# XiYe20/VPTR

Measured on AMD Instinct MI355X. Metric: predicted frames/sec (train step) NAR KTH 10->10 @64x64, higher is better.
Workload: dtype bf16x3 (split-bf16 MFMA, fp32 accumulate/storage); 1 GPU; K64: KTH 64x64x1 10->10, VPTREnc/Dec(528, Tanh, reflect) + VPTRFormerNAR(4 enc + 8 dec, d=528, 8 heads, ws 4, dropout 0.10), single_iter of train_NAR.py, random-init weights; per_gpu_batch=16, global_batch=16, frames_per_clip=10, parallelism=dp1, launch=hipGraph, dec_weight_grads=True, frozen_encoder_convs=winograd F(4x4,3x3), 36 strided-batch P16 products per convolution

## Files before the change

### vptr_amd/csrc/gemm_p16.hip

```cpp
#include "gemm_shared.h"

#include <atomic>

typedef __attribute__((ext_vector_type(4))) short s16x4;
typedef __attribute__((ext_vector_type(8))) short s16x8;

constexpr int P16_STAGE = 40 * 1024;

#define P16_GLDS(laddr, gptr) \
  asm volatile("s_mov_b32 m0, %0\n\tglobal_load_lds_dwordx4 %1, off" ::"s"(__builtin_amdgcn_readfirstlane(laddr)), "v"(gptr) : "memory")

__global__ __launch_bounds__(256) void to_p16_kernel(const float* __restrict__ x, unsigned char* __restrict__ out, int64_t n4) {
  for (int64_t i = (int64_t)blockIdx.x * 256 + threadIdx.x; i < n4; i += (int64_t)gridDim.x * 256) {
    const float4 v = reinterpret_cast<const float4*>(x)[i];
    vptr_p16_store4(out, i * 4, v);
  }
}
extern "C" int vptr_to_p16(const float* x, void* out, int64_t rows, int C, vptr_stream_t stream) {
  VPTR_CHECK(x && out && rows > 0 && C > 0 && C % 16 == 0, "to_p16: C must be a positive multiple of 16 (got %d)", C);
  VPTR_CHECK(((reinterpret_cast<uintptr_t>(x) | reinterpret_cast<uintptr_t>(out)) & 15) == 0, "to_p16: pointers must be 16-byte aligned");
  const int64_t n4 = rows * C / 4;
  to_p16_kernel<<<(unsigned)hmin64((n4 + 255) / 256, 16384), 256, 0, (hipStream_t)stream>>>(x, reinterpret_cast<unsigned char*>(out), n4);
  VPTR_LAUNCH_CHECK();
  return 0;
// ... 132 lines not shown

  f32x4 acc[2][6];
#pragma unroll
  for (int mi = 0; mi < 2; ++mi)
#pragma unroll
    for (int ni = 0; ni < 6; ++ni) acc[mi][ni] = (f32x4){0.f, 0.f, 0.f, 0.f};
  int offAh[2], offBh[6];
  const int ch = (lq >> 1) * 4 + (lq & 1);
#pragma unroll
  for (int mi = 0; mi < 2; ++mi) {
    const int r = wm * 32 + mi * 16 + lr, f = (r >> 1) & 7;
    offAh[mi] = r * 128 + ((ch ^ f) << 4);
  }
#pragma unroll
  for (int ni = 0; ni < 6; ++ni) {
    const int r = (wn * 6 + ni) * 16 + lr, f = (r >> 1) & 7;
    offBh[ni] = 16384 + r * 128 + ((ch ^ f) << 4);
  }
  const int nkt = nk * nseg;
  if (NST == 2) issue(0, 0);
  for (int kt = 0; kt < nkt; ++kt) {
    if (NST == 2) __builtin_amdgcn_s_waitcnt(0x0f70);
    __syncthreads();
    if (NST == 2 && kt + 1 < nkt) issue(kt + 1, (kt + 1) & 1);
    const unsigned char* st = p16_smem + (kt & (NST - 1)) * P16_STAGE;
    bf16x8 ah[2], al[2];
#pragma unroll
    for (int mi = 0; mi < 2; ++mi) {
      ah[mi] = *reinterpret_cast<const bf16x8*>(st + offAh[mi]);
      al[mi] = *reinterpret_cast<const bf16x8*>(st + (offAh[mi] ^ 32));
    }
    if (ktail) {
      const int sg = (int)(kt >= nk) + (int)(kt >= 2 * nk);
      if (kt - sg * nk == nk - 1 && lq >= 2) {
#pragma unroll
        for (int mi = 0; mi < 2; ++mi) {
          ah[mi] = (bf16x8){0, 0, 0, 0, 0, 0, 0, 0};
          al[mi] = (bf16x8){0, 0, 0, 0, 0, 0, 0, 0};
        }
      }
    }
    bf16x8 bh[2], bl[2];
    bh[0] = *reinterpret_cast<const bf16x8*>(st + offBh[0]);
    bl[0] = *reinterpret_cast<const bf16x8*>(st + (offBh[0] ^ 32));
#pragma unroll
    for (int ni = 0; ni < 6; ++ni) {
      if (ni == 5 && wn == 1) break;
      if (ni + 1 < 6 && !(ni + 1 == 5 && wn == 1)) {
        bh[(ni + 1) & 1] = *reinterpret_cast<const bf16x8*>(st + offBh[ni + 1]);
        bl[(ni + 1) & 1] = *reinterpret_cast<const bf16x8*>(st + (offBh[ni + 1] ^ 32));
      }
      __builtin_amdgcn_sched_barrier(0);
#pragma unroll
      for (int mi = 0; mi < 2; ++mi) {
        acc[mi][ni] = __builtin_amdgcn_mfma_f32_16x16x32_bf16(al[mi], bh[ni & 1], acc[mi][ni], 0, 0, 0);
        acc[mi][ni] = __builtin_amdgcn_mfma_f32_16x16x32_bf16(ah[mi], bl[ni & 1], acc[mi][ni], 0, 0, 0);
        acc[mi][ni] = __builtin_amdgcn_mfma_f32_16x16x32_bf16(ah[mi], bh[ni & 1], acc[mi][ni], 0, 0, 0);
      }
      __builtin_amdgcn_sched_barrier(0);
    }
  }
  constexpr bool LEAN = EPI != 0;
  if (LEAN) {
    __syncthreads();
    gemm_epilogue_rows_halves_batched<NFN, EPI>(p, mb, acc, reinterpret_cast<float*>(p16_smem), m0, n0, wm, wn, lr, lq, tid, true, false);
  } else if (NST == 4 && !p.atomic && epi_vec_ok(p)) {
    __syncthreads();
    gemm_epilogue_rows_halves_batched<NFN, 0>(p, mb, acc, reinterpret_cast<float*>(p16_smem), m0, n0, wm, wn, lr, lq, tid, true, false);
  } else if (!p.atomic && epi_vec_ok(p)) {
    __syncthreads();
    gemm_epilogue_rows_halves<NFN>(p, mb, acc, reinterpret_cast<float*>(p16_smem), m0, n0, wm, wn, lr, lq, tid, true, false);
  } else {
    gemm_epilogue_serial<NFN>(p, mb, acc, m0, n0, wm, wn, lr, lq, true, p.atomic != 0);
  }
}

__device__ __forceinline__ bf16x8 p16_tr_frag(const unsigned char* st, const int off, const int rb0) {
  const s16x4 a = __builtin_amdgcn_ds_read_tr16_b64_v4i16((__attribute__((address_space(3))) s16x4*)(st + off + rb0));
  const s16x4 b = __builtin_amdgcn_ds_read_tr16_b64_v4i16((__attribute__((address_space(3))) s16x4*)(st + off + (128 - rb0)));
  const s16x8 c = __builtin_shufflevector(a, b, 0, 1, 2, 3, 4, 5, 6, 7);
  return __builtin_bit_cast(bf16x8, c);
}

struct WgSync {
  int* cnt;
  int base;
  int n;
  bool live;
};

template <int SYNC, int MI>
__device__ __forceinline__ void wgrad_p16_tile(const vptr_gemm_desc& p, const int tile, unsigned char* p16_smem, WgSync& sy) {
  constexpr int NW = 8, BN = 176, WM = NW / 2, TR = 16 * MI * WM;
  constexpr int PA = TR / 8 / NW, PB = 24 / NW;
  constexpr int AREG = TR * 128, STG = AREG + 24 * 1024;
  const int NG = p.M, KX = p.N, T = p.K;
  const int tiles_n = (KX + BN - 1) / BN;
  const int m0 = (tile / tiles_n) * TR, n0 = (tile % tiles_n) * BN;
  const int tid = threadIdx.x, lane = tid & 63, wave = tid >> 6;
  const int wm = wave % WM, wn = wave / WM, lr = lane & 15, lq = lane >> 4;
  const int nk = (T + 31) >> 5;
  const int64_t pg = p.lda * 4, px = p.ldb * 4;
  const unsigned char* Gb = reinterpret_cast<const unsigned char*>(p.A);
  const unsigned char* Xb = reinterpret_cast<const unsigned char*>(p.B);

  int colA[PA], colB[PB], trow[PA + PB];
  {
    const int ms = lane >> 4, half = lane & 1, t = (lane & 15) >> 1;
#pragma unroll
    for (int i = 0; i < PA; ++i) {
      const int u = wave + NW * i;
      const int gran = min((m0 >> 4) + (u >> 2) * 2 + (ms >> 1), (NG >> 4) - 1);
      colA[i] = gran * 64 + (ms & 1) * 32 + half * 16;
      trow[i] = (u & 3) * 8 + t;
    }
#pragma unroll
    for (int i = 0; i < PB; ++i) {
      const int v = wave + NW * i;
      const int gran = min((n0 >> 4) + (v >> 2) * 2 + (ms >> 1), (KX >> 4) - 1);
      colB[i] = gran * 64 + (ms & 1) * 32 + half * 16;
      trow[PA + i] = (v & 3) * 8 + t;
    }
  }
  auto issue = [&](const int kt, const int stage) {
    const int t0 = kt * 32;
#pragma unroll
    for (int i = 0; i < PA; ++i)
      P16_GLDS((uint32_t)(stage * STG + (wave + NW * i) * 1024), Gb + (int64_t)min(t0 + trow[i], T - 1) * pg + colA[i]);
#pragma unroll
    for (int i = 0; i < PB; ++i)
      P16_GLDS((uint32_t)(stage * STG + AREG + (wave + NW * i) * 1024), Xb + (int64_t)min(t0 + trow[PA + i], T - 1) * px + colB[i]);
  };

  f32x4 acc[MI][6];
#pragma unroll
  for (int mi = 0; mi < MI; ++mi)
#pragma unroll
    for (int ni = 0; ni < 6; ++ni) acc[mi][ni] = (f32x4){0.f, 0.f, 0.f, 0.f};
  const int lane_off = lq * 1024 + (lr >> 2) * 32 + (lr & 3) * 8;
  const int rb0 = (lq & 1) * 128;
  int offA[MI], offB[6];
#pragma unroll
  for (int mi = 0; mi < MI; ++mi) {
    const int f = wm * MI + mi;
    offA[mi] = (f >> 1) * 4096 + (f & 1) * 512 + lane_off;
  }
#pragma unroll
  for (int ni = 0; ni < 6; ++ni) {
    const int f = wn * 6 + ni;
    offB[ni] = AREG + (f >> 1) * 4096 + (f & 1) * 512 + lane_off;
  }
  const bool flip = p.d_transposed != 0;
  const bool want_rowsum = !flip && p.a_rowsum != nullptr && n0 == 0 && wn == 1;
  const int f0 = (NG - m0 + 15) >> 4;
  const bool colsum_wave = flip && p.a_rowsum != nullptr && f0 < TR / 16 && wm == f0 / MI;
  const int cmi = f0 - wm * MI;
  const __bf16 one = (__bf16)1.0f, zero = (__bf16)0.0f;
  const bf16x8 ones = {one, one, one, one, one, one, one, one};
  const bf16x8 zeros = {zero, zero, zero, zero, zero, zero, zero, zero};
  const bool ttail = (T & 31) != 0;
  const bool rows_live = m0 + wm * (16 * MI) < NG;

  issue(0, 0);
  for (int kt = 0; kt < nk; ++kt) {
    if (SYNC > 0 && kt > 0 && (kt & (SYNC / 2 - 1)) == 0 && threadIdx.x == 0) {
      const int ph = kt & (SYNC - 1);
      if (ph == 0) __hip_atomic_fetch_add(sy.cnt, 1, __ATOMIC_RELAXED, __HIP_MEMORY_SCOPE_AGENT);
      else if (kt > SYNC && sy.live) {
        const int target = sy.base + (kt / SYNC) * sy.n;
        int spins = 0;
        while (__hip_atomic_load(sy.cnt, __ATOMIC_RELAXED, __HIP_MEMORY_SCOPE_AGENT) < target) {
          if (++spins > 3000) {
            sy.live = false;
            __hip_atomic_fetch_add(sy.cnt + 48, 1, __ATOMIC_RELAXED, __HIP_MEMORY_SCOPE_AGENT);
            break;
          }
          __builtin_amdgcn_s_sleep(8);
        }
      }
    }
    __builtin_amdgcn_s_waitcnt(0x0f70);
    __syncthreads();
    if (kt + 1 < nk) issue(kt + 1, (kt + 1) & 1);
    if (!rows_live && !colsum_wave) continue;
    const unsigned char* st = p16_smem + (kt & 1) * STG;
    bf16x8 ah[MI], al[MI];
#pragma unroll
    for (int mi = 0; mi < MI; ++mi) {
      ah[mi] = p16_tr_frag(st, offA[mi], rb0);
      al[mi] = p16_tr_frag(st, offA[mi] + 256, rb0);
    }
    if (colsum_wave) {
#pragma unroll
      for (int mi = 0; mi < MI; ++mi)
        if (mi == cmi) { ah[mi] = ones; al[mi] = zeros; }
    }
    if (ttail && kt == nk - 1) {
      const int tv = T - kt * 32;
#pragma unroll
      for (int e = 0; e < 8; ++e) {
        const int tok = 8 * lq + 4 * ((e >> 2) ^ (lq & 1)) + (e & 3);
        if (tok >= tv) {
#pragma unroll
          for (int mi = 0; mi < MI; ++mi) { ah[mi][e] = zero; al[mi][e] = zero; }
        }
      }
    }
    bf16x8 bh[2], bl[2];
    bh[0] = p16_tr_frag(st, offB[0], rb0);
    bl[0] = p16_tr_frag(st, offB[0] + 256, rb0);
#pragma unroll
    for (int ni = 0; ni < 6; ++ni) {
      if (ni == 5 && wn == 1 && !want_rowsum) break;
      if (ni + 1 < 6) {
        if (ni + 1 == 5 && wn == 1) {
          bh[(ni + 1) & 1] = ones;
          bl[(ni + 1) & 1] = zeros;
        } else {
          bh[(ni + 1) & 1] = p16_tr_frag(st, offB[ni + 1], rb0);
          bl[(ni + 1) & 1] = p16_tr_frag(st, offB[ni + 1] + 256, rb0);
        }
      }
      __builtin_amdgcn_sched_barrier(0);
#pragma unroll
      for (int mi = 0; mi < MI; ++mi) {
        acc[mi][ni] = __builtin_amdgcn_mfma_f32_16x16x32_bf16(al[mi], bh[ni & 1], acc[mi][ni], 0, 0, 0);
        acc[mi][ni] = __builtin_amdgcn_mfma_f32_16x16x32_bf16(ah[mi], bl[ni & 1], acc[mi][ni], 0, 0, 0);
        acc[mi][ni] = __builtin_amdgcn_mfma_f32_16x16x32_bf16(ah[mi], bh[ni & 1], acc[mi][ni], 0, 0, 0);
      }
      __builtin_amdgcn_sched_barrier(0);
    }
  }
  const float alpha = p.alpha;
#pragma unroll
  for (int ni = 0; ni < 6; ++ni) {
    const int nf = wn * 6 + ni, col = n0 + nf * 16 + lr;
    if (nf < 11 && col < KX) {
#pragma unroll
      for (int mi = 0; mi < MI; ++mi)
#pragma unroll
        for (int r = 0; r < 4; ++r) {
          const int row = m0 + (wm * MI + mi) * 16 + lq * 4 + r;
          if (row < NG) {
            float* dst = flip ? p.D + (int64_t)col * p.ldd + row : p.D + (int64_t)row * p.ldd + col;
            if (p.atomic) unsafeAtomicAdd(dst, acc[mi][ni][r] * alpha);
            else *dst = acc[mi][ni][r] * alpha;
          }
        }
    }
  }
  if (colsum_wave && lq == 0) {
#pragma unroll
    for (int ni = 0; ni < 6; ++ni) {
      const int nf = wn * 6 + ni, col = n0 + nf * 16 + lr;
      if (nf < 11 && col < KX) {
        float cs = 0.f;
#pragma unroll
        for (int mi = 0; mi < MI; ++mi)
          if (mi == cmi) cs = acc[mi][ni][0];
        unsafeAtomicAdd(p.a_rowsum + col, cs * alpha);
      }
    }
  }
  if (want_rowsum && lr == 0) {
#pragma unroll
    for (int mi = 0; mi < MI; ++mi)
#pragma unroll
      for (int r = 0; r < 4; ++r) {
        const int row = m0 + (wm * MI + mi) * 16 + lq * 4 + r;
        if (row < NG) unsafeAtomicAdd(p.a_rowsum + row, acc[mi][5][r] * alpha);
      }
  }
}


template <int NSTAGE, int TAG = 0, int NW = 8, int MI = 16 / NW>
__global__ __launch_bounds__(64 * NW, MI == 2 ? 4 : 2) void vptr_wgrad_p16_kernel(const vptr_gemm_desc* __restrict__ descs, const int* __restrict__ tile_start,
                                                                            const int count) {
  static_assert(NSTAGE == 2 && NW == 8, "two stages, eight waves");
  extern __shared__ __attribute__((aligned(1024))) unsigned char p16_smem[];
  const int lg = xcd_logical_block();
  int lo = 0, hi = count - 1;
  while (lo < hi) {
    const int mid = (lo + hi + 1) >> 1;
    if (tile_start[mid] <= lg) lo = mid;
    else hi = mid - 1;
  }
  WgSync none = {nullptr, 0, 0, false};
  wgrad_p16_tile<0, MI>(descs[lo], lg - tile_start[lo], p16_smem, none);
}

__device__ int g_wgrad_sync_ws[8 * 64];
template <int S, int NW = 8, int MI = 16 / NW, int NST = 2>
__global__ __launch_bounds__(64 * NW, MI == 2 ? 4 : 2) void vptr_wgrad_p16_sync_kernel(const vptr_gemm_desc* __restrict__ descs, const int* __restrict__ tile_start,
                                                                const int count, const int total_tiles) {
  static_assert(NST == 2 && NW == 8, "two stages, eight waves");
  extern __shared__ __attribute__((aligned(1024))) unsigned char p16_smem[];
  int* const ws = g_wgrad_sync_ws;
  const int xcd = blockIdx.x & 7, slot = blockIdx.x >> 3, slots = gridDim.x >> 3;
  const int xq = total_tiles >> 3, xr = total_tiles & 7;
  const int first = xcd * xq + min(xcd, xr), mine = xq + (xcd < xr ? 1 : 0);
  const int nk = (descs[0].K + 31) >> 5;
  const int per_tile = (nk - 1) / S;
  WgSync sy = {ws + xcd * 64, 0, 0, true};
  for (int r = 0; r * slots + slot < mine; ++r) {
    const int lg = first + r * slots + slot;
    int lo = 0, hi = count - 1;
    while (lo < hi) {
      const int mid = (lo + hi + 1) >> 1;
      if (tile_start[mid] <= lg) lo = mid;
      else hi = mid - 1;
    }
    sy.base = r * slots * per_tile;
    sy.n = min(slots, mine - r * slots);
    if (r > 0) __syncthreads();
    wgrad_p16_tile<S, MI>(descs[lo], lg - tile_start[lo], p16_smem, sy);
  }
  if (threadIdx.x == 0) {
    int* done = ws + xcd * 64 + 32;
    if (__hip_atomic_fetch_add(done, 1, __ATOMIC_RELAXED, __HIP_MEMORY_SCOPE_AGENT) == slots - 1) {
      __hip_atomic_store(ws + xcd * 64, 0, __ATOMIC_RELAXED, __HIP_MEMORY_SCOPE_AGENT);
      __hip_atomic_store(done, 0, __ATOMIC_RELAXED, __HIP_MEMORY_SCOPE_AGENT);
    }
  }
}

__global__ void wgrad_sync_stats_kernel(int* __restrict__ out) {
  if (threadIdx.x < 8) out[threadIdx.x] = g_wgrad_sync_ws[threadIdx.x * 64 + 48];
}
extern "C" int vptr_wgrad_sync_stats(int* out_dev, vptr_stream_t stream) {
  VPTR_CHECK(out_dev != nullptr, "wgrad_sync_stats: null output");
// ... 31 lines not shown
  if (d.alpha == 0.f) d.alpha = 1.f;
  if (d.batch < 1) d.batch = 1;
  if (d.ksegs < 1) d.ksegs = 1;
  const bool strided = d.batch_stride_d != 0;
  if (strided)
    VPTR_CHECK(d.ksegs == 1 && d.batch <= 4096 && !d.Dpre && !d.residual && !d.atomic && !d.batch_accum && !d.frame_stats && !d.act_grad_src && !d.rowscale &&
                   !d.colscale && d.dropout_p == 0.f && d.act == VPTR_ACT_NONE && !d.act_after &&
                   ((d.batch_stride_a | d.batch_stride_b | d.batch_stride_d) & 15) == 0 && d.batch_stride_a >= 0 && d.batch_stride_b >= 0 && d.batch_stride_d > 0,
               "vptr_gemm(p16): a strided batch takes bias / alpha only and strides that are non-negative multiples of 16");
  VPTR_CHECK((strided || d.batch <= 3) && d.ksegs <= 3 && (d.batch == 1 || d.ksegs == 1), "vptr_gemm(p16): at most 3 batch members or 3 K segments");
  uintptr_t bits = reinterpret_cast<uintptr_t>(d.A) | reinterpret_cast<uintptr_t>(d.B);
  const int extra = strided ? 0 : (d.batch > 1 ? d.batch : d.ksegs) - 1;
  if (extra >= 1) {
    VPTR_CHECK(d.A_x1 && d.B_x1, "vptr_gemm(p16): member / segment 1 needs A_x1, B_x1");
    bits |= reinterpret_cast<uintptr_t>(d.A_x1) | reinterpret_cast<uintptr_t>(d.B_x1);
  }
  if (extra >= 2) {
    VPTR_CHECK(d.A_x2 && d.B_x2, "vptr_gemm(p16): member / segment 2 needs A_x2, B_x2");
    bits |= reinterpret_cast<uintptr_t>(d.A_x2) | reinterpret_cast<uintptr_t>(d.B_x2);
  }
  VPTR_CHECK((bits & 63) == 0, "vptr_gemm(p16): operands must be 64-byte aligned (whole granules)");
  if (d.batch > 1 && !strided) {
    VPTR_CHECK(d.D_x1 && (d.batch < 3 || d.D_x2) && !d.Dpre && !d.residual && !d.atomic, "vptr_gemm(p16): bad batch members");
    if (d.alpha_x1 == 0.f) d.alpha_x1 = 1.f;
    if (d.alpha_x2 == 0.f) d.alpha_x2 = 1.f;
  }
  if (d.rowscale) VPTR_CHECK(d.rs_div >= 1 && d.rs_mod >= 1, "vptr_gemm: rowscale needs rs_div, rs_mod >= 1");
  if (d.dropout_p > 0.f) VPTR_CHECK(d.seed_dev != nullptr && d.dropout_p < 1.f, "vptr_gemm: dropout needs seed_dev and p < 1");
  if (d.d_p16)
    VPTR_CHECK(!d.atomic && d.N % 16 == 0 && d.ldd % 16 == 0 && (d.ldr & 3) == 0 &&
                   ((reinterpret_cast<uintptr_t>(d.D) | reinterpret_cast<uintptr_t>(d.D_x1) | reinterpret_cast<uintptr_t>(d.D_x2)) & 63) == 0 &&
                   ((reinterpret_cast<uintptr_t>(d.residual) | reinterpret_cast<uintptr_t>(d.bias) | reinterpret_cast<uintptr_t>(d.colscale) |
                     reinterpret_cast<uintptr_t>(d.Dpre) | reinterpret_cast<uintptr_t>(d.bias_x1) | reinterpret_cast<uintptr_t>(d.bias_x2)) & 15) == 0,
               "vptr_gemm(p16): a P16 output needs N, ldd multiples of 16, 64-byte aligned D and 16-byte aligned epilogue operands, no atomics");
  static bool attr_set = false;
  if (!attr_set) {
    if (!p16_reserve_lds<0>() || !p16_reserve_lds<1>() || !p16_reserve_lds<2>() || !p16_reserve_lds<3>() || !p16_reserve_lds<4>()) {
      vptr_set_error("vptr_gemm(p16): cannot reserve %d bytes of LDS", 4 * P16_STAGE);
      return -1;
    }
    attr_set = true;
  }
  const int tiles = ((d.M + GBM - 1) / GBM) * ((d.N + 175) / 176) * d.batch;
  uintptr_t ebits = reinterpret_cast<uintptr_t>(d.D) | reinterpret_cast<uintptr_t>(d.residual) | reinterpret_cast<uintptr_t>(d.bias);
  if (d.batch > 1 && !strided) ebits |= reinterpret_cast<uintptr_t>(d.D_x1) | reinterpret_cast<uintptr_t>(d.D_x2) | reinterpret_cast<uintptr_t>(d.bias_x1) | reinterpret_cast<uintptr_t>(d.bias_x2);
  const bool lean = !d.colscale && !d.Dpre && !d.rowscale && d.act == VPTR_ACT_NONE && d.dropout_p == 0.f && !d.act_after && !d.atomic &&
                    (ebits & 15) == 0 && (d.N & 3) == 0 && (d.ldd & 3) == 0 && (d.ldr & 3) == 0;
  const bool lean3 = !lean && !d.colscale && !d.Dpre && (d.rowscale || d.dropout_p > 0.f) && d.act == VPTR_ACT_NONE &&
                     !d.act_after && !d.atomic && !d.frame_stats && (ebits & 15) == 0 && (d.N & 3) == 0 && (d.ldd & 3) == 0 && (d.ldr & 3) == 0;
  const bool lean4 = !lean && !lean3 && !d.colscale && !d.rowscale && !d.residual && !d.act_after && !d.atomic &&
                     d.act != VPTR_ACT_NONE && !d.act_grad_src && !d.frame_stats && d.batch == 1 && !d.batch_accum &&
                     ((ebits | reinterpret_cast<uintptr_t>(d.Dpre)) & 15) == 0 && (d.N & 3) == 0 && (d.ldd & 3) == 0;
  const bool lone = tiles <= vptr_cu_count();
  if (d.frame_stats)
    VPTR_CHECK(d.frame_rows >= 64 && d.frame_rows % 64 == 0 && d.M % 64 == 0 && !d.act_grad_src && lean && d.batch == 1,
               "vptr_gemm(p16): frame_stats needs frame_rows %% 64 == 0, M %% 64 == 0 and a plain launch (bias / alpha / residual only)");
  if (d.act_grad_src) {
    VPTR_CHECK(!d.colscale && !d.Dpre && !d.rowscale && !d.residual && !d.bias && !d.act_after && !d.atomic && d.batch == 1 && d.ksegs == 1 &&
                   d.act != VPTR_ACT_NONE && ((ebits | reinterpret_cast<uintptr_t>(d.act_grad_src)) & 15) == 0 && (d.N & 3) == 0 && (d.ldd & 3) == 0,
               "vptr_gemm(p16): act_grad_src combines with alpha / dropout / P16 output only and needs 16-byte aligned operands, N, ldd multiples of 4");
    p16_launch<2>(d, tiles, lone, st);
    return 0;
  }
  if (d.batch_accum)
    VPTR_CHECK(lean && d.batch > 1 && !d.d_p16 && (d.batch_accum >> d.batch) == 0, "vptr_gemm(p16): batch_accum is an option of plain fp32-output batch launches");
  if (lean4) p16_launch<4>(d, tiles, lone, st);
  else if (lean3) p16_launch<3>(d, tiles, lone, st);
  else if (lean) p16_launch<1>(d, tiles, lone, st);
  else p16_launch<0>(d, tiles, lone, st);
  return 0;
}

static std::atomic<int> g_wgrad_launches[5];
extern "C" int vptr_wgrad_kernel_counts(int* out_host, int n) {
  VPTR_CHECK(out_host != nullptr && n >= 1 && n <= 5, "wgrad_kernel_counts: n must be 1 .. 5 (got %d)", n);
  for (int i = 0; i < n; ++i) out_host[i] = g_wgrad_launches[i].load(std::memory_order_relaxed);
  return 0;
}

int vptr_wgrad_p16_launch(const vptr_gemm_desc* proto, const vptr_gemm_desc* descs_dev, const int* tile_start_dev, int count, int total_tiles,
                          hipStream_t st) {
  VPTR_CHECK(proto->b_mode == VPTR_B_P16T && proto->precision == 3, "vptr_gemm_grouped(p16): both operands token-major P16, precision 3");
  VPTR_CHECK(proto->split_k >= -3, "vptr_gemm_grouped(p16): unknown split_k code %d (include/vptr_hip.h)", proto->split_k);
  constexpr int STG256 = 256 * 128 + 24 * 1024;
  static int sync = -1;
  if (sync < 0) {
    if (hipFuncSetAttribute(reinterpret_cast<const void*>(&vptr_wgrad_p16_kernel<2>), hipFuncAttributeMaxDynamicSharedMemorySize, 2 * P16_STAGE) != hipSuccess ||
        hipFuncSetAttribute(reinterpret_cast<const void*>(&vptr_wgrad_p16_kernel<2, 1>), hipFuncAttributeMaxDynamicSharedMemorySize, 2 * P16_STAGE) != hipSuccess ||
        hipFuncSetAttribute(reinterpret_cast<const void*>(&vptr_wgrad_p16_kernel<2, 0, 8, 4>), hipFuncAttributeMaxDynamicSharedMemorySize, 2 * STG256) != hipSuccess) {
      vptr_set_error("vptr_gemm_grouped(p16): cannot reserve LDS");
      return -1;
    }
    const char* e = getenv("VPTR_WGRAD_SYNC");
    sync = !(e && atoi(e) == 0);
    int per_cu = 0;
    if (sync && (hipFuncSetAttribute(reinterpret_cast<const void*>(&vptr_wgrad_p16_sync_kernel<16>), hipFuncAttributeMaxDynamicSharedMemorySize, 2 * P16_STAGE) != hipSuccess ||
                 hipFuncSetAttribute(reinterpret_cast<const void*>(&vptr_wgrad_p16_sync_kernel<16, 8, 4>), hipFuncAttributeMaxDynamicSharedMemorySize, 2 * STG256) != hipSuccess ||
                 hipOccupancyMaxActiveBlocksPerMultiprocessor(&per_cu, vptr_wgrad_p16_sync_kernel<16>, GNT, 2 * P16_STAGE) != hipSuccess || per_cu < 2))
      sync = 0;
  }
  const int cus = vptr_cu_count();
  if (proto->split_k == -2 || proto->split_k == -3) {
    VPTR_CHECK(proto->atomic, "vptr_gemm_grouped(p16): 256-row tiles accumulate with atomics only");
    if (proto->split_k == -2 && sync && total_tiles >= 512 && cus > 0 && cus % 8 == 0) {
      vptr_wgrad_p16_sync_kernel<16, 8, 4><<<cus, GNT, 2 * STG256, st>>>(descs_dev, tile_start_dev, count, total_tiles);
      g_wgrad_launches[4].fetch_add(1, std::memory_order_relaxed);
    } else {
      vptr_wgrad_p16_kernel<2, 0, 8, 4><<<total_tiles, GNT, 2 * STG256, st>>>(descs_dev, tile_start_dev, count);
      g_wgrad_launches[3].fetch_add(1, std::memory_order_relaxed);
    }
    return 0;
  }
  if (sync && proto->split_k == -1 && proto->atomic && total_tiles >= 1024 && cus > 0 && cus % 4 == 0) {
    vptr_wgrad_p16_sync_kernel<16><<<2 * cus, GNT, 2 * P16_STAGE, st>>>(descs_dev, tile_start_dev, count, total_tiles);
    g_wgrad_launches[2].fetch_add(1, std::memory_order_relaxed);
  } else if (!proto->atomic) {
    vptr_wgrad_p16_kernel<2, 1><<<total_tiles, GNT, 2 * P16_STAGE, st>>>(descs_dev, tile_start_dev, count);
    g_wgrad_launches[1].fetch_add(1, std::memory_order_relaxed);
  } else {
    vptr_wgrad_p16_kernel<2><<<total_tiles, GNT, 2 * P16_STAGE, st>>>(descs_dev, tile_start_dev, count);
    g_wgrad_launches[0].fetch_add(1, std::memory_order_relaxed);
  }
  return 0;
}
```

### vptr_amd/ops/__init__.py

```python
from .core import (
    ACT_NONE, ACT_GELU, ACT_RELU, ACT_LRELU, PAD_MODES, _Config, config, set_deterministic, _direct_apply, _seed_state, _seed_scope,
    _dev_key, _master_seed, new_seed_scope, seed_tensor, manual_seed, DROPPATH_SITE0, droppath_scales, _c, gemm_raw, _Profiling,
    profiling, gemm_nfn, A_P16, B_P16, A_P16T, B_P16T, p16_ok, to_p16, _AsP16Fn, _AsP16Fn_apply, as_p16, p16_decode,
)
from .wgrad import (
    _wgrad_q, defer_wgrad, take_wgrads, requeue_wgrads, discard_wgrads, _reduce_q, defer_partial_reduce, flush_partial_reduces,
    _wgrad_hold, hold_wgrads, _auto_flush_wgrads, _pin_pool, _pin_pool_small,
    _wgrad_tune, _graph_keepalive, _graph_reserve, _upload_stats, reserve_graph_staging, _to_device_async, _wgrad_tune_book, _wgrad_tune_decide, _TUNE_SAMPLES, wgrad_tune_open,
    wgrad_tune_settle, plan_wgrad_launches, _launch_wgrad_group, convt_weight_grads, flush_wgrads, _split_k_for,
)
from .grads import (
    _flat_slabs, register_flat_slab, unregister_flat_slabs, unregister_flat_slab, flat_grad_for, _grad_arenas, _storage_refs, _GradArena,
    _register_grad_arena, _arm_grad_arena, _arena_grad_for, _engine_accumulates_into, _acc_nodes, _drop_acc_nodes, _loose_grad_for,
    grad_dest_for, _bw_blocks, _BW_BLOCK, _bw_zeros,
)
from .planes import (
    WeightPlanes, _wplane_stores, _wplane_cache, _WPLANE_CACHE_BYTES, register_weight_planes, ensure_module_planes,
    invalidate_weight_planes, weight_planes_for, linear_weights_of,
)
from .linear import (
    _linear_param_grads, _LinearFn, _LinearFn_apply, linear, frame_stats_ok, _zero_arena, zero_arena, FRAME_STATS_STRIDE, frame_stats_buffer, _MlpFn,
    _MlpFn_apply, mlp,
)
from .norm import (
    _LayerNormFn, _LayerNormFn_apply, layernorm, _AddRowTabFn, _AddRowTabFn_apply, add_rowtab,
)
from .attention import (
    _winattn_workspace, _WinAttnFn, _WinAttnFn_apply, window_attention, _TAttnFn, _TAttnFn_apply, temporal_attention, KVGradAccum,
    _ProjAttnFn, _ProjAttnFn_apply, _proj_attention, proj_window_attention, proj_temporal_attention, proj_temporal_attention_step, _TSAttnFn,
    temporal_spatial_window_attention,
)
from .convffn import (
    _norm_act_backward, _NormActFn, _NormActFn_apply, norm_act, _DWConvFn, _DWConvFn_apply, dwconv3x3, norm_dwconv_ok, _NormDWConvFn,
    _NormDWConvFn_apply, norm_dwconv3x3,
)
from .layout import (
    _WindowCopyFn, _WindowCopyFn_apply, pad_tokens, crop_tokens, _ToTokensFn, _ToTokensFn_apply, _FromTokensFn, _FromTokensFn_apply,
    nchw_to_tokens, tokens_to_nchw,
)
from .conv import (
    SubpixelWeights, conv_weight_as_gemm_b, in_flat_slab, weights_cacheable, frozen_weights, conv_nhwc, split_planes,
    conv_weight_as_planes, conv_nhwc_planes, wino_ok, wino_filter, wino_buffers, wino_in, wino_gemm, wino_out, wino_fused_ok, wino_out_in, wino_conv3x3,
    wino_resnet_blocks, _Conv2dNHWCFn, conv2d_nhwc, _Conv7InFn, conv7_in, _Conv7OutFn, conv7_out, bn_fold,
)
from .losses import (
    _MseGdlFn, mse_gdl, _NceFn, nce_loss,
)
from .metrics import (
    FRAME_METRICS_BAND, FRAME_METRICS_MAX_W, frame_metrics,
)
from .ingest import (
    INGEST_MAX_OUT, INGEST_MAX_KSIZE, ingest_clips,
)
from .panels import (
    PANELS_MAX_CLIPS, clip_panels, pad_indices, panel_shape,
)
from . import core, planes, wgrad, grads, linear, norm, attention, convffn, layout, conv, losses, metrics, ingest, panels
from .._lib import lib
```

### vptr_amd/ops/core.py

```python
import ctypes
import os

import torch

from .._lib import GemmDesc, check, lib, ptr, stream


ACT_NONE, ACT_GELU, ACT_RELU, ACT_LRELU = 0, 1, 2, 3
PAD_MODES = {"zero": 0, "reflect": 1, "replicate": 2}


class _Config:
    gemm_precision = 3
    group_wgrads = True
    group_loose_wgrads = os.environ.get("VPTR_LOOSE_WGRADS", "1") != "0"
    defer_ln_param_grads = os.environ.get("VPTR_DEFER_LN", "1") != "0"
    wgrad_flip = os.environ.get("VPTR_WGRAD_FLIP", "1") != "0"
    wgrad_token_split = os.environ.get("VPTR_WGRAD_TOKEN_SPLIT", "1") != "0"
    wgrad_rows = (lambda v: v if v == "auto" else int(v))(os.environ.get("VPTR_WGRAD_ROWS", "auto"))
    subpixel_convt = os.environ.get("VPTR_SUBPIXEL_CONVT", "1") != "0"
    weights_frozen = False
    use_p16 = os.environ.get("VPTR_P16", "1") != "0"
    fused_mlp = os.environ.get("VPTR_FUSED_MLP", "1") != "0"
    fused_frame_stats = os.environ.get("VPTR_FUSED_STATS", "1") != "0"
    winograd = os.environ.get("VPTR_ENC_WINOGRAD", "1") != "0"
    winograd_fuse = os.environ.get("VPTR_WINO_FUSE", "1") != "0"
    fused_norm_dwconv_mode = int(os.environ.get("VPTR_FUSED_NORM_DW", "1") or 1)
    loose_grad_arena = os.environ.get("VPTR_GRAD_ARENA", "1") != "0"
    deterministic = False


config = _Config()


def set_deterministic(on=True):
    on = bool(on)
    if on and not config.deterministic:
        config._fused_before = config.fused_frame_stats
        config.fused_frame_stats = False
    elif not on and config.deterministic:
        config.fused_frame_stats = getattr(config, "_fused_before", True)
    config.deterministic = on
    lib.vptr_set_deterministic(int(on))


if os.environ.get("VPTR_DETERMINISTIC") == "1":
    set_deterministic(True)


def _direct_apply(fn_cls):
    return super(torch.autograd.Function, fn_cls).apply

_seed_state = {}
_seed_scope = {}


def _dev_key(device):
    return torch.device(device).index or 0


def _master_seed(device):
    key = _dev_key(device)
    if key not in _seed_state:
        if torch.distributed.is_available() and torch.distributed.is_initialized():
            rank = torch.distributed.get_rank()
        else:
            rank = int(os.environ.get("RANK", "0"))
        v = (torch.initial_seed() * 0x9E3779B97F4A7C15 + (rank + 1) * 0xBF58476D1CE4E5B9 + (key + 1) * 0x94D049BB133111EB) & 0x7FFFFFFFFFFFFFFF
        _seed_state[key] = torch.full((1,), v, dtype=torch.int64, device=device)
    return _seed_state[key]


def new_seed_scope(device):
    m = _master_seed(device)
    m.add_(0x9E3779B9)
    snap = m.clone()
    _seed_scope[_dev_key(device)] = snap
    return snap


def seed_tensor(device):
    key = _dev_key(device)
    if key not in _seed_scope:
        return new_seed_scope(device)
    return _seed_scope[key]


def manual_seed(device, value):
    _master_seed(device).fill_(int(value))
    _seed_scope.pop(_dev_key(device), None)


DROPPATH_SITE0 = 0x44500000


def droppath_scales(keep, maxcount, device, site_offset=0):
    out = torch.empty((keep.shape[0], int(maxcount)), device=device, dtype=torch.float32)
    check(lib.vptr_droppath_scales(ptr(keep), ptr(out), keep.shape[0], int(maxcount), ptr(seed_tensor(device)),
                                   DROPPATH_SITE0 + int(site_offset), stream()), "vptr_droppath_scales")
    return out

# ... 142 lines not shown
```

### vptr_amd/ops/wgrad.py

```python
import ctypes
import os

import torch

from .. import _lib
from .._lib import GemmDesc, check, lib, ptr, stream
from .core import A_P16T, B_P16T, config, profiling, to_p16


_wgrad_q = []


def defer_wgrad(g, x, dW, N, K, M, db=None, alpha=1.0, p16=False):
    _wgrad_q.append((g, x, dW, N, K, M, config.gemm_precision, db, float(alpha), bool(p16)))
    try:
        torch.autograd.Variable._execution_engine.queue_callback(_auto_flush_wgrads)
    except RuntimeError:
        pass


def take_wgrads():
    items = list(_wgrad_q)
    del _wgrad_q[:]
    return items
# ... 123 lines not shown
    tune["choice"] = min(best, key=best.get) if best else 128
    tune["ms"] = best


def _wgrad_tune_book(tune):
    r_, e0_, e1_ = tune["pending"]
    tune["samples"][r_].append(e0_.elapsed_time(e1_))
    tune["pending"] = None
    _wgrad_tune_decide(tune)


def wgrad_tune_open():
    return any(t["choice"] is None for t in _wgrad_tune.values())


def wgrad_tune_settle():
    if any(t["pending"] is not None for t in _wgrad_tune.values()):
        torch.cuda.synchronize()
    for t in _wgrad_tune.values():
        if t["pending"] is not None:
            _wgrad_tune_book(t)
        if t["choice"] is None:
            _wgrad_tune_decide(t, final=True)


def plan_wgrad_launches(probs, cols, p16, atomic, allow_sync, rows_mode, token_split=True):
    subs = []
    for (ap, bp, dp, rp, lda, ldb, ldd, rows_, cols_, M, alpha, flip) in probs:
        small_group = p16 and atomic and token_split and len(probs) <= 3
        if p16 and atomic and rows_mode == 256 and not small_group and rows_ >= 1024 and (rows_ // 256) * 256 >= 0.85 * rows_:
            full = (rows_ // 256) * 256
            rem256 = rows_ - full
            subs.append((ap, bp, dp, 0 if (flip and rem256) else rp, lda, ldb, ldd, full, cols_, M, alpha, flip, 256))
            if rem256:
                subs.append((ap + full * 4, bp, dp + (full * 4 if flip else full * ldd * 4), (rp + (0 if flip else full * 4)) if rp else 0,
                             lda, ldb, ldd, rem256, cols_, M, alpha, flip, 128))
            continue
        subs.append((ap, bp, dp, rp, lda, ldb, ldd, rows_, cols_, M, alpha, flip))

    def trows(sub):
        return sub[12] if len(sub) > 12 else 128

    def tiles_of(sub):
        return ((sub[7] + trows(sub) - 1) // trows(sub)) * ((sub[8] + cols - 1) // cols)
    if p16 and atomic and token_split:
        tot = sum(tiles_of(x) for x in subs)
        if 0 < tot < 384:
            want = (512 + tot - 1) // tot
            cut = []
            for sub in subs:
                Mtok = sub[9]
                S = max(1, min(want, Mtok // 1024))
                if S == 1:
                    cut.append(sub)
                    continue
                chunk = (((Mtok + S - 1) // S + 31) // 32) * 32
                t0 = 0
                while t0 < Mtok:
                    n_t = min(chunk, Mtok - t0)
                    cut.append((sub[0] + t0 * sub[4] * 4, sub[1] + t0 * sub[5] * 4) + tuple(sub[2:9]) + (n_t,) + tuple(sub[10:]))
                    t0 += n_t
            subs = cut
    tall = [x for x in subs if trows(x) != 128]
    subs = [x for x in subs if trows(x) == 128]
    launches = [(subs, False)] if subs else []
    if allow_sync and p16 and atomic:
        classes = {}
        for sub in subs:
            classes.setdefault(sub[9], []).append(sub)
        if len(classes) == 1:
            launches = [(subs, True)]
        elif classes:
            big = [(t, c) for t, c in classes.items() if sum(tiles_of(x) for x in c) >= 1024]
            rest = [x for t, c in classes.items() if sum(tiles_of(y) for y in c) < 1024 for x in c]
            launches = [(c, True) for _, c in sorted(big, key=lambda tc: -tc[0])] + ([(rest, False)] if rest else [])
    if tall:
        tclasses = {}
        for sub in tall:
            tclasses.setdefault(sub[9], []).append(sub)
        launches = [(c, bool(allow_sync)) for _, c in sorted(tclasses.items(), key=lambda tc: -tc[0])] + launches
    return launches


def _launch_wgrad_group(its, atomic=1, allow_sync=True):
    groups = {}
    for it in its:
        p16 = it[9]
        groups.setdefault((176 if p16 else int(lib.vptr_gemm_tile_cols(it[4])), it[6], p16), []).append(it)
    for (cols, prec, p16), grp in groups.items():
        rows_mode = config.wgrad_rows
        tune = None
        if rows_mode == "auto":
            rows_mode = 128
            if p16 and atomic and len(grp) > 3:
                sig = (allow_sync,) + tuple(sorted((it[3], it[4], it[5]) for it in grp))
                tune = _wgrad_tune.setdefault(sig, {"samples": {128: [], 256: []}, "ms": {}, "pending": None, "choice": None})
                capturing = torch.cuda.is_current_stream_capturing()
                if not capturing and tune["pending"] is not None and tune["pending"][2].query():
                    _wgrad_tune_book(tune)
                if tune["choice"] is not None:
                    rows_mode, tune = tune["choice"], None
                elif capturing or tune["pending"] is not None:
                    known = {r: min(v[1:] or v) for r, v in tune["samples"].items() if v}
                    rows_mode, tune = (min(known, key=known.get) if known else 128), None
                else:
                    rows_mode = 128 if len(tune["samples"][128]) <= len(tune["samples"][256]) else 256
        probs = []
        flops = 0.0
        for (g, x, dW, N, K, M, _, db, alpha, _p) in grp:
            flops += 2.0 * M * N * K
            flip = (p16 and config.wgrad_flip and N < K and N % 176 == 0 and K % 128 != 0 and 128 - K % 128 >= 32)
            if flip:
                a, b, rows_, cols_, lda, ldb = x, g, K, N, x.stride(0), g.stride(0)
            else:
                a, b, rows_, cols_, lda, ldb = g, x, N, K, g.stride(0), x.stride(0)
            ap, bp, dp, rp, ldd = a.data_ptr(), b.data_ptr(), dW.data_ptr(), (db.data_ptr() if db is not None else 0), dW.stride(0)
            probs.append((ap, bp, dp, rp, lda, ldb, ldd, rows_, cols_, M, alpha, flip))
        launches = plan_wgrad_launches(probs, cols, p16, atomic, allow_sync, rows_mode,
                                       token_split=config.wgrad_token_split and not config.deterministic)

        def trows(sub):
            return sub[12] if len(sub) > 12 else 128

        def tiles_of(sub):
            return ((sub[7] + trows(sub) - 1) // trows(sub)) * ((sub[8] + cols - 1) // cols)
        dev = grp[0][0].device
        import struct
        if tune is not None:
            t_e0, t_e1 = torch.cuda.Event(enable_timing=True), torch.cuda.Event(enable_timing=True)
            t_e0.record()
        for lsubs, vouch in launches:
            n = len(lsubs)
            descs = (GemmDesc * n)()
            starts = []
            total = 0
            lflops = 0.0
            tr = trows(lsubs[0])
            for i, sub in enumerate(lsubs):
                (ap, bp, dp, rp, lda, ldb, ldd, rows_, cols_, M, alpha, flip) = sub[:12]
                d = descs[i]
                d.precision, d.split_k, d.atomic, d.alpha = prec, 1, int(atomic), alpha
                d.A, d.B, d.D, d.a_rowsum = ap, bp, dp, (rp or None)
                d.lda, d.ldb, d.ldd = lda, ldb, ldd
                d.M, d.N, d.K = rows_, cols_, M
                d.d_transposed = int(flip)
                d.a_mode, d.b_mode = (A_P16T, B_P16T) if p16 else (1, 1)
                starts.append(total)
                total += tiles_of(lsubs[i])
                lflops += 2.0 * rows_ * cols_ * M
            if tr == 256:
                descs[0].split_k = -2 if vouch else -3
            elif vouch:
                descs[0].split_k = -1
            raw = _to_device_async(bytes(descs), dev)
            st = _to_device_async(struct.pack("%di" % len(starts), *starts), dev)
            prof = profiling.gemm
            if prof is not None:
                e0, e1 = torch.cuda.Event(enable_timing=True), torch.cuda.Event(enable_timing=True)
                e0.record()
            check(lib.vptr_gemm_grouped(ctypes.byref(descs[0]), ptr(raw), ptr(st), n, total, stream()), "vptr_gemm_grouped")
            if prof is not None:
                e1.record()
                sync = p16 and atomic and vouch and total >= (512 if tr != 128 else 1024) and os.environ.get("VPTR_WGRAD_SYNC", "16") not in ("0", "")
                prof.append(((cols // 16, prec, 6 if p16 else 1, 4 if p16 else 1, (("grouped_sync%d" % tr if tr != 128 else "grouped_sync") if sync else "grouped") if atomic else "grouped_split"),
                             lflops, e0, e1))
        if tune is not None:
            t_e1.record()
            tune["pending"] = (rows_mode, t_e0, t_e1)


def convt_weight_grads(layers, tokens_per_split=2560):
    items, keep, outs, red = [], [], [], []
    for (x, g, B, ih, iw, ci, oh, ow, co) in layers:
        pix = B * ih * iw
        P = torch.empty((pix, 9 * co), device=g.device, dtype=torch.float32)
        check(lib.vptr_im2col_nhwc_p16(ptr(g), ptr(P), B, oh, ow, co, ih, iw, 3, 3, 2, 1, 0, stream()), "vptr_im2col_nhwc_p16")
        xs = to_p16(x)
        S = max(1, pix // int(tokens_per_split))
        step = (pix + S - 1) // S
        step = (step + 31) // 32 * 32
        S = (pix + step - 1) // step
        part = torch.empty((S, ci, 9 * co), device=g.device, dtype=torch.float32)
        for k in range(S):
            r0, r1 = k * step, min(pix, (k + 1) * step)
            items.append((xs[r0:r1], P[r0:r1], part[k], ci, 9 * co, r1 - r0, config.gemm_precision, None, 1.0, True))
        D = torch.zeros((ci, 9 * co), device=g.device, dtype=torch.float32)
        red.append((part, D, S, ci * 9 * co))
        keep += [P, xs, part]
        outs.append(D)
    _launch_wgrad_group(items, atomic=0)
    tab = (_lib.ReduceEntry * len(red))()
    for i, (part, D, S, C) in enumerate(red):
        tab[i].part, tab[i].dst0, tab[i].dst1, tab[i].nparts, tab[i].C = ptr(part), ptr(D), None, S, C
    raw = _to_device_async(bytes(tab), outs[0].device)
    esz = ctypes.sizeof(_lib.ReduceEntry)
    for i, (part, D, S, C) in enumerate(red):
        check(lib.vptr_partial_reduce(ctypes.c_void_p(raw.data_ptr() + i * esz), 1, C, 1, stream()), "vptr_partial_reduce")
    return outs


def flush_wgrads(chunks=1, on_chunk=None):
    flush_partial_reduces()
    if not _wgrad_q:
        if on_chunk is not None:
            on_chunk(None)
        return
    items = list(_wgrad_q)
    del _wgrad_q[:]
    if chunks <= 1 or len(items) < 2 * chunks:
        items.sort(key=lambda it: (-it[3] * it[4], it[1].data_ptr(), it[2].data_ptr()))
        _launch_wgrad_group(items)
        if on_chunk is not None:
            on_chunk(None)
        return
    items.sort(key=lambda it: it[2].data_ptr())
    work = [float(it[3]) * it[4] for it in items]
    per = sum(work) / chunks
    acc, lo = 0.0, 0
    bounds = []
    for i, w in enumerate(work):
        acc += w
        if acc >= per * (len(bounds) + 1) and len(bounds) < chunks - 1 and i + 1 < len(items):
            bounds.append(i + 1)
    bounds.append(len(items))
# ... 12 lines not shown
```

Before: 3720 frames/s.

## Use vectorized non-atomic RMW for non-overlapping wgrad outputs; skip dead A loads

The host now checks which weight-gradient outputs in a grouped P16 wgrad launch have non-overlapping destination ranges (including rowsum buffers). Those get a new mode 2, in which the kernel replaces per-element scalar atomic adds with float4 read-modify-write. For the non-flipped layout it first stages each 16-row fragment through an LDS patch so the global accesses are coalesced. Separately, the kernel skips global-to-LDS loads of A rows that lie beyond NG. The risk is that plain RMW is only correct if no two tiles or launches add into the same output concurrently, which relies on the host overlap check being complete.

```diff
diff --git a/vptr_amd/csrc/gemm_p16.hip b/vptr_amd/csrc/gemm_p16.hip
--- a/vptr_amd/csrc/gemm_p16.hip
+++ b/vptr_amd/csrc/gemm_p16.hip
@@ -238,6 +238,12 @@
   return __builtin_bit_cast(bf16x8, c);
 }
 
+__device__ __forceinline__ float wgrad_scaled(const float a, const float alpha) {
+  float x = a * alpha;
+  asm volatile("" : "+v"(x));
+  return x;
+}
+
 struct WgSync {
   int* cnt;
   int base;
@@ -278,11 +284,17 @@
       trow[PA + i] = (v & 3) * 8 + t;
     }
   }
+  unsigned live = 0;
+#pragma unroll
+  for (int i = 0; i < PA; ++i)
+    if (m0 + 32 * ((wave + NW * i) >> 2) < NG) live |= 1u << i;
+  const unsigned amask = __builtin_amdgcn_readfirstlane(live);
   auto issue = [&](const int kt, const int stage) {
     const int t0 = kt * 32;
 #pragma unroll
     for (int i = 0; i < PA; ++i)
-      P16_GLDS((uint32_t)(stage * STG + (wave + NW * i) * 1024), Gb + (int64_t)min(t0 + trow[i], T - 1) * pg + colA[i]);
+      if (amask >> i & 1)
+        P16_GLDS((uint32_t)(stage * STG + (wave + NW * i) * 1024), Gb + (int64_t)min(t0 + trow[i], T - 1) * pg + colA[i]);
 #pragma unroll
     for (int i = 0; i < PB; ++i)
       P16_GLDS((uint32_t)(stage * STG + AREG + (wave + NW * i) * 1024), Xb + (int64_t)min(t0 + trow[PA + i], T - 1) * px + colB[i]);
@@ -388,21 +400,80 @@
     }
   }
   const float alpha = p.alpha;
-#pragma unroll
-  for (int ni = 0; ni < 6; ++ni) {
-    const int nf = wn * 6 + ni, col = n0 + nf * 16 + lr;
-    if (nf < 11 && col < KX) {
-#pragma unroll
-      for (int mi = 0; mi < MI; ++mi)
-#pragma unroll
-        for (int r = 0; r < 4; ++r) {
-          const int row = m0 + (wm * MI + mi) * 16 + lq * 4 + r;
+  const bool vec_rmw = p.atomic == 2 && (reinterpret_cast<uintptr_t>(p.D) & 15) == 0 && (p.ldd & 3) == 0 && ((flip ? NG : KX) & 3) == 0;
+  if (vec_rmw && flip) {
+#pragma unroll
+    for (int ni = 0; ni < 6; ++ni) {
+      const int nf = wn * 6 + ni, col = n0 + nf * 16 + lr;
+      if (nf < 11 && col < KX) {
+#pragma unroll
+        for (int mi = 0; mi < MI; ++mi) {
+          const int row = m0 + (wm * MI + mi) * 16 + lq * 4;
           if (row < NG) {
-            float* dst = flip ? p.D + (int64_t)col * p.ldd + row : p.D + (int64_t)row * p.ldd + col;
-            if (p.atomic) unsafeAtomicAdd(dst, acc[mi][ni][r] * alpha);
-            else *dst = acc[mi][ni][r] * alpha;
+            float4* dst = reinterpret_cast<float4*>(p.D + (int64_t)col * p.ldd + row);
+            float4 v = *dst;
+            v.x += wgrad_scaled(acc[mi][ni][0], alpha);
+            v.y += wgrad_scaled(acc[mi][ni][1], alpha);
+            v.z += wgrad_scaled(acc[mi][ni][2], alpha);
+            v.w += wgrad_scaled(acc[mi][ni][3], alpha);
+            *dst = v;
           }
         }
+      }
+    }
+  } else if (vec_rmw) {
+    constexpr int PLD = 100;
+    __syncthreads();
+    float* patch = reinterpret_cast<float*>(p16_smem) + wave * (16 * PLD);
+    const int ncol = wn == 1 ? 80 : 96;
+#pragma unroll
+    for (int mi = 0; mi < MI; ++mi) {
+      const int row0 = m0 + (wm * MI + mi) * 16;
+      if (row0 < NG) {
+#pragma unroll
+        for (int ni = 0; ni < 6; ++ni)
+#pragma unroll
+          for (int r = 0; r < 4; ++r) patch[(lq * 4 + r) * PLD + ni * 16 + lr] = acc[mi][ni][r] * alpha;
+        __builtin_amdgcn_fence(__ATOMIC_RELEASE, "wavefront");
+        __builtin_amdgcn_wave_barrier();
+        __builtin_amdgcn_fence(__ATOMIC_ACQUIRE, "wavefront");
+#pragma unroll
+        for (int j = 0; j < 6; ++j) {
+          const int idx = lane + 64 * j, pr = idx / 24, pc = (idx % 24) * 4;
+          const int row = row0 + pr, col = n0 + wn * 96 + pc;
+          if (row < NG && pc < ncol && col < KX) {
+            const float4 a = *reinterpret_cast<const float4*>(patch + pr * PLD + pc);
+            float4* dst = reinterpret_cast<float4*>(p.D + (int64_t)row * p.ldd + col);
+            float4 v = *dst;
+            v.x += a.x;
+            v.y += a.y;
+            v.z += a.z;
+            v.w += a.w;
+            *dst = v;
+          }
+        }
+        __builtin_amdgcn_fence(__ATOMIC_RELEASE, "wavefront");
+        __builtin_amdgcn_wave_barrier();
+        __builtin_amdgcn_fence(__ATOMIC_ACQUIRE, "wavefront");
+      }
+    }
+  } else {
+#pragma unroll
+    for (int ni = 0; ni < 6; ++ni) {
+      const int nf = wn * 6 + ni, col = n0 + nf * 16 + lr;
+      if (nf < 11 && col < KX) {
+#pragma unroll
+        for (int mi = 0; mi < MI; ++mi)
+#pragma unroll
+          for (int r = 0; r < 4; ++r) {
+            const int row = m0 + (wm * MI + mi) * 16 + lq * 4 + r;
+            if (row < NG) {
+              float* dst = flip ? p.D + (int64_t)col * p.ldd + row : p.D + (int64_t)row * p.ldd + col;
+              if (p.atomic) unsafeAtomicAdd(dst, acc[mi][ni][r] * alpha);
+              else *dst = acc[mi][ni][r] * alpha;
+            }
+          }
+      }
     }
   }
   if (colsum_wave && lq == 0) {
@@ -600,6 +671,7 @@
                           hipStream_t st) {
   VPTR_CHECK(proto->b_mode == VPTR_B_P16T && proto->precision == 3, "vptr_gemm_grouped(p16): both operands token-major P16, precision 3");
   VPTR_CHECK(proto->split_k >= -3, "vptr_gemm_grouped(p16): unknown split_k code %d (include/vptr_hip.h)", proto->split_k);
+  VPTR_CHECK(proto->atomic >= 0 && proto->atomic <= 2, "vptr_gemm_grouped(p16): atomic must be 0, 1 or 2 (got %d)", proto->atomic);
   constexpr int STG256 = 256 * 128 + 24 * 1024;
   static int sync = -1;
   if (sync < 0) {
diff --git a/vptr_amd/ops/__init__.py b/vptr_amd/ops/__init__.py
--- a/vptr_amd/ops/__init__.py
+++ b/vptr_amd/ops/__init__.py
@@ -7,7 +7,7 @@
     _wgrad_q, defer_wgrad, take_wgrads, requeue_wgrads, discard_wgrads, _reduce_q, defer_partial_reduce, flush_partial_reduces,
     _wgrad_hold, hold_wgrads, _auto_flush_wgrads, _pin_pool, _pin_pool_small,
     _wgrad_tune, _graph_keepalive, _graph_reserve, _upload_stats, reserve_graph_staging, _to_device_async, _wgrad_tune_book, _wgrad_tune_decide, _TUNE_SAMPLES, wgrad_tune_open,
-    wgrad_tune_settle, plan_wgrad_launches, _launch_wgrad_group, convt_weight_grads, flush_wgrads, _split_k_for,
+    wgrad_tune_settle, plan_wgrad_launches, wgrad_atomic_modes, _launch_wgrad_group, convt_weight_grads, flush_wgrads, _split_k_for,
 )
 from .grads import (
     _flat_slabs, register_flat_slab, unregister_flat_slabs, unregister_flat_slab, flat_grad_for, _grad_arenas, _storage_refs, _GradArena,
diff --git a/vptr_amd/ops/core.py b/vptr_amd/ops/core.py
--- a/vptr_amd/ops/core.py
+++ b/vptr_amd/ops/core.py
@@ -17,6 +17,7 @@
     defer_ln_param_grads = os.environ.get("VPTR_DEFER_LN", "1") != "0"
     wgrad_flip = os.environ.get("VPTR_WGRAD_FLIP", "1") != "0"
     wgrad_token_split = os.environ.get("VPTR_WGRAD_TOKEN_SPLIT", "1") != "0"
+    wgrad_vec_add = os.environ.get("VPTR_WGRAD_VEC_ADD", "1") != "0"
     wgrad_rows = (lambda v: v if v == "auto" else int(v))(os.environ.get("VPTR_WGRAD_ROWS", "auto"))
     subpixel_convt = os.environ.get("VPTR_SUBPIXEL_CONVT", "1") != "0"
     weights_frozen = False
diff --git a/vptr_amd/ops/wgrad.py b/vptr_amd/ops/wgrad.py
--- a/vptr_amd/ops/wgrad.py
+++ b/vptr_amd/ops/wgrad.py
@@ -229,6 +229,29 @@
     return launches
 
 
+def wgrad_atomic_modes(subs, atomic, p16):
+    if not (p16 and atomic == 1):
+        return [int(atomic)] * len(subs)
+    spans = []
+    for i, sub in enumerate(subs):
+        (_, _, dp, rp, _, _, ldd, rows_, cols_, _, _, flip) = sub[:12]
+        h, w = (cols_, rows_) if flip else (rows_, cols_)
+        spans.append((dp, dp + 4 * ((h - 1) * ldd + w), i))
+        if rp:
+            spans.append((rp, rp + 4 * h, -1))
+    spans.sort()
+    modes = [2] * len(subs)
+    end, owner = -1, None
+    for lo, hi, i in spans:
+        if lo < end:
+            for j in (i, owner):
+                if j >= 0:
+                    modes[j] = 1
+        if hi > end:
+            end, owner = hi, i
+    return modes
+
+
 def _launch_wgrad_group(its, atomic=1, allow_sync=True):
     groups = {}
     for it in its:
@@ -283,10 +306,11 @@
             total = 0
             lflops = 0.0
             tr = trows(lsubs[0])
+            modes = wgrad_atomic_modes(lsubs, int(atomic), p16) if config.wgrad_vec_add else [int(atomic)] * n
             for i, sub in enumerate(lsubs):
                 (ap, bp, dp, rp, lda, ldb, ldd, rows_, cols_, M, alpha, flip) = sub[:12]
                 d = descs[i]
-                d.precision, d.split_k, d.atomic, d.alpha = prec, 1, int(atomic), alpha
+                d.precision, d.split_k, d.atomic, d.alpha = prec, 1, modes[i], alpha
                 d.A, d.B, d.D, d.a_rowsum = ap, bp, dp, (rp or None)
                 d.lda, d.ldb, d.ldd = lda, ldb, ldd
                 d.M, d.N, d.K = rows_, cols_, M
```

Measured after the change: 3741 frames/s (median of 6 runs). About the same (+0.6%).
